# JuliaHealth/Thunderbolt.jl

Measured on AMD Instinct MI355X. Metric: element-integrations/sec + DoF-updates/sec, 10M-hex Q1 monodomain, higher is better.
Workload: dtype f64

## Files before the change

include/tbhip.h:

```cpp
#ifndef TBHIP_H
#define TBHIP_H
#include <stddef.h>
#include <stdint.h>

#ifdef __cplusplus
extern "C" {
#endif

typedef struct tb_device tb_device;
typedef struct tb_mesh tb_mesh;
typedef struct tb_pattern tb_pattern;
typedef struct tb_form tb_form;
typedef struct tb_locator tb_locator;
typedef struct tb_ecg tb_ecg;

enum {
    TB_OK = 0,
    TB_ERR_BAD_ARG = -1,
    TB_ERR_HIP = -2,
    TB_ERR_NEG_DETJ = -3,
    TB_ERR_PATTERN = -4,
    TB_ERR_UNSUPPORTED = -5,
    TB_ERR_NOMEM = -6
};
// ... 249 lines not shown
                     double *d_S);
int tb_gather_indexed(tb_device *dev, int64_t n, const double *d_vec, const int32_t *d_idx, double *d_out);
int tb_extract_diagonal(tb_pattern *pat, const double *d_nzval, double *d_diag);
int tb_scatter_add_indexed(tb_device *dev, int64_t n, const double *d_in, const int32_t *d_idx, double *d_vec);
int tb_scatter_indexed(tb_device *dev, int64_t n, const double *d_in, const int32_t *d_idx, double *d_vec);
typedef struct tb_comm tb_comm;
#define TB_COMM_ID_BYTES 128
enum { TB_REDUCE_SUM = 0, TB_REDUCE_MAX = 1 };
int tb_comm_unique_id(void *id128);
int tb_comm_create(tb_device *dev, const void *id128, int rank, int world_size, tb_comm **out);
int tb_comm_destroy(tb_comm *comm);
int tb_comm_rank_size(tb_comm *comm, int *rank, int *size);
int tb_comm_exchange(tb_comm *comm, int n_peers, const int32_t *peers, const int64_t *counts, const double *const *d_send, double *const *d_recv);
int tb_comm_allreduce(tb_comm *comm, double *d_buf, int64_t n, int op);
int tb_comm_exchange_begin(tb_comm *comm, int n_peers, const int32_t *peers, const int64_t *counts, const double *const *d_send, double *const *d_recv);
int tb_comm_exchange_end(tb_comm *comm);
typedef struct tb_graph tb_graph;
int tb_graph_begin(tb_device *dev);
int tb_graph_end(tb_device *dev, tb_graph **out);
int tb_graph_launch(tb_graph *graph, double t);
int tb_graph_node_count(tb_graph *graph, int *n);
int tb_graph_destroy(tb_graph *graph);
int tb_pattern_patch_stats(tb_pattern *pat, int64_t *out6);
int tb_pattern_spmv_plan(tb_pattern *pat, int64_t *out2);
int tb_spmv_mirror(tb_pattern *pat, const double *d_nzval);
int tb_spmv_csr_rows(tb_pattern *pat, const double *d_nzval, const double *d_x, int64_t n_rows, const int32_t *d_rows, double *d_out);
int tb_spmv_csr_dot(tb_pattern *pat, const double *d_nzval, const double *d_x, double *d_y, double *d_dot);
int tb_apply_zero_csr(tb_pattern *pat, double *d_nzval, double *d_f, const uint8_t *d_prescribed, double diag);
int tb_meandiag(tb_pattern *pat, const double *d_nzval, double *result);
int tb_max(tb_device *dev, int64_t n, const double *d_x, int64_t stride, double *result);

int tb_newmark_predict(tb_device *dev, int64_t n, double dt, double beta, double gamma, const double *d_u, const double *d_v, const double *d_a,
                       double *d_utilde, double *d_vtilde);
int tb_newmark_stage(tb_pattern *pat, const double *d_Mnz, double c, const double *d_u, const double *d_utilde, double *d_Jnz, double *d_r);
int tb_newmark_correct(tb_device *dev, int64_t n, double dt, double beta, double gamma, const double *d_u, const double *d_utilde, const double *d_vtilde,
                       double *d_a, double *d_v);
int tb_hermite_interpolate(tb_device *dev, int64_t n, double theta, double dt, int derivative, const double *d_u0, const double *d_v0, const double *d_u1,
                           const double *d_v1, double *d_out);

int tb_convert_f64_to_f32(tb_device *dev, int64_t n, const double *d_in, float *d_out);
int tb_convert_f32_to_f64(tb_device *dev, int64_t n, const float *d_in, double *d_out);
int tb_assemble_matrix_f32(tb_form *form, tb_pattern *pat, int strategy, double t, float *d_nzval);
int tb_assemble_matrix_pair_f32(tb_form *mass, tb_form *diffusion, tb_pattern *pat, int strategy, double t, float *d_nzval_mass, float *d_nzval_diffusion);
int tb_assemble_vector_f32(tb_form *form, int strategy, double t, float *d_b);
int tb_reaction_step_f32(tb_device *dev, int model, const double *params, int n_params, float *d_u, float *d_du, int64_t n_points, int n_states, int layout,
                         const float *d_x, int sdim, double t, double dt, int substeps, double threshold);
// ... 23 lines not shown
```

thunderbolt.jl_amd/_lib.py:

```python
import ctypes as C
import os
import subprocess

_HERE = os.path.dirname(os.path.abspath(__file__))
LIB_PATH = os.environ.get("TB_LIBTBHIP") or os.path.join(_HERE, "libtbhip.so")

TB_OK = 0
TB_ERR_BAD_ARG, TB_ERR_HIP, TB_ERR_NEG_DETJ, TB_ERR_PATTERN, TB_ERR_UNSUPPORTED, TB_ERR_NOMEM = -1, -2, -3, -4, -5, -6
TB_QUAD4, TB_HEX8, TB_TET4, TB_HEX27, TB_TET10 = 2, 3, 4, 5, 6
TB_STRATEGY_ATOMIC, TB_STRATEGY_PER_COLOR, TB_STRATEGY_ELEMENT, TB_STRATEGY_PATCH = 0, 1, 2, 3
TB_FORM_MASS, TB_FORM_DIFFUSION, TB_FORM_SOURCE, TB_FORM_HYPERELASTIC = 0, 1, 2, 3
TB_MATERIAL_HOLZAPFEL_OGDEN_2009 = 0
TB_BC_ROBIN, TB_BC_NORMAL_SPRING, TB_BC_PRESSURE, TB_BC_BENDING_SPRING, TB_BC_PRESSURE_FIELD = 0, 1, 2, 3, 4
TB_VOLUME_RSAFDQ2022, TB_VOLUME_HIRSCHVOGEL2017 = 0, 1
TB_COEF_CONST_SCALAR, TB_COEF_CONST_TENSOR, TB_COEF_FIELD_SCALAR = 0, 1, 2
TB_COEF_SPECTRAL_CONST, TB_COEF_SPECTRAL_FIELD, TB_COEF_TRANSVERSE_CONST = 3, 4, 5
TB_SRC_CONST, TB_SRC_NORM_PLUS_T, TB_SRC_COS_EXP, TB_SRC_TABULATED = 0, 1, 2, 3
TB_CELL_FHN, TB_CELL_ALIEV_PANFILOV, TB_CELL_PCG2019, TB_CELL_TT06, TB_CELL_FHN_HETEROGENEOUS, TB_CELL_ORD11 = 0, 1, 2, 3, 4, 5
TB_LAYOUT_SOA, TB_LAYOUT_AOS = 0, 1

c_dp = C.POINTER(C.c_double)
c_i32p = C.POINTER(C.c_int32)
c_i64p = C.POINTER(C.c_int64)
vp = C.c_void_p
# ... 147 lines not shown
    "tb_heat_matrix_f32": (C.c_int, [vp, C.c_int64, vp, vp, C.c_double, vp]),
    "tb_axpy_f32": (C.c_int, [vp, C.c_int64, C.c_double, vp, vp]),
    "tb_cg_solve_f32": (C.c_int, [vp, vp, vp, vp, C.c_double, C.c_double, C.c_int, C.c_int, vp, vp]),
    "tb_extract_diagonal": (C.c_int, [vp, vp, vp]),
    "tb_pattern_patch_stats": (C.c_int, [vp, vp]),
    "tb_comm_unique_id": (C.c_int, [vp]),
    "tb_comm_create": (C.c_int, [vp, vp, C.c_int, C.c_int, C.POINTER(vp)]),
    "tb_comm_destroy": (C.c_int, [vp]),
    "tb_comm_rank_size": (C.c_int, [vp, vp, vp]),
    "tb_comm_exchange": (C.c_int, [vp, C.c_int, vp, vp, vp, vp]),
    "tb_comm_allreduce": (C.c_int, [vp, vp, C.c_int64, C.c_int]),
    "tb_comm_exchange_begin": (C.c_int, [vp, C.c_int, vp, vp, vp, vp]),
    "tb_cgd_iteration": (C.c_int, [vp, vp, vp, vp, vp, vp, vp, vp]),
    "tb_cg1_update": (C.c_int, [vp, C.c_int64, vp, vp, vp, vp, vp, vp, vp, vp, vp]),
    "tb_cg1_fold": (C.c_int, [vp, vp]),
    "tb_cg1_iteration": (C.c_int, [vp, vp, vp, vp, vp, vp, vp, vp, vp, vp]),
    "tb_graph_begin": (C.c_int, [vp]),
    "tb_graph_end": (C.c_int, [vp, C.POINTER(vp)]),
    "tb_graph_launch": (C.c_int, [vp, C.c_double]),
    "tb_graph_node_count": (C.c_int, [vp, C.POINTER(C.c_int)]),
    "tb_graph_destroy": (C.c_int, [vp]),
    "tb_comm_exchange_end": (C.c_int, [vp]),
    "tb_pattern_spmv_plan": (C.c_int, [vp, vp]),
    "tb_scatter_add_indexed": (C.c_int, [vp, C.c_int64, vp, vp, vp]),
    "tb_scatter_indexed": (C.c_int, [vp, C.c_int64, vp, vp, vp]),
    "tb_spmv_csr_rows": (C.c_int, [vp, vp, vp, C.c_int64, vp, vp]),
    "tb_spmv_csr_dot": (C.c_int, [vp, vp, vp, vp, vp]),
    "tb_spmv_mirror": (C.c_int, [vp, vp]),
    "tb_apply_zero_csr": (C.c_int, [vp, vp, vp, vp, C.c_double]),
    "tb_meandiag": (C.c_int, [vp, vp, C.POINTER(C.c_double)]),
    "tb_max": (C.c_int, [vp, C.c_int64, vp, C.c_int64, C.POINTER(C.c_double)]),
    "tb_host_generate_grid_hex": (C.c_int, [C.c_int, C.c_int, C.c_int, c_dp, c_dp, c_dp, c_i32p]),
    "tb_host_generate_grid_tet": (C.c_int, [C.c_int, C.c_int, C.c_int, c_dp, c_dp, c_dp, c_i32p]),
    "tb_host_generate_grid_quad": (C.c_int, [C.c_int, C.c_int, c_dp, c_dp, c_dp, c_i32p]),
    "tb_host_perturb_nodes": (C.c_int, [C.c_int, C.c_int, C.c_int, C.c_double, c_dp]),
    "tb_host_close_dofs": (C.c_int64, [C.c_int, C.c_int, C.c_int64, C.c_int64, c_i32p, c_i32p]),
    "tb_host_build_pattern": (C.c_int64, [C.c_int64, C.c_int, c_i32p, C.c_int64, c_i64p, c_i32p]),
    "tb_host_locality_permutation": (C.c_int, [C.c_int, C.c_int64, c_dp, C.c_int64, c_i32p, C.c_int, c_i32p, C.c_int64, C.c_int, c_i32p, c_i32p, c_i32p]),
}


class TBError(RuntimeError):
    def __init__(self, code, msg):
        super().__init__("libtbhip error %d: %s" % (code, msg))
        self.code = code

# ... 42 lines not shown
```

thunderbolt.jl_amd/csrc/tb_api.cpp:

```cpp
#include <algorithm>
#include <mutex>
#include <cmath>
#include <cstdarg>
#include <cstring>

#include <omp.h>

#include "tb_internal.h"

namespace tb {

static thread_local std::string g_error;

void set_error(const char *fmt, ...)
{
    char buf[1024];
    va_list ap;
    va_start(ap, fmt);
    vsnprintf(buf, sizeof buf, fmt, ap);
    va_end(ap);
    g_error = buf;
}

static thread_local std::string g_last_kernel;
// ... 1268 lines not shown

int tb_pattern_spmv_plan(tb_pattern *pat, int64_t *out2)
{
    TB_REQUIRE(pat && out2, "tb_pattern_spmv_plan: NULL argument");
    TB_HIP(hipSetDevice(pat->mesh->dev->id));
    int rc = spmv_plans(pat);
    if (rc) return rc;
    out2[0] = pat->n_sig; out2[1] = pat->sig_entries;
    return TB_OK;
}

int tb_pattern_patch_stats(tb_pattern *pat, int64_t *out6)
{
    TB_REQUIRE(pat && out6, "tb_pattern_patch_stats: NULL argument");
    TB_HIP(hipSetDevice(pat->mesh->dev->id));
    int rc = ensure_patch_plans(pat->mesh, nullptr);
    if (rc) return rc;
    const PatchPlan *pp = pat->mesh->patches.get();
    out6[0] = pp->n_patches; out6[1] = pp->total_elems; out6[2] = pat->mesh->n_cells; out6[3] = pp->max_elems; out6[4] = pp->max_rows;
    out6[5] = pat->patch_fused ? (int64_t)pat->patch_fused->max_lds_entries * 8 : (pat->patch_mat ? (int64_t)pat->patch_mat->max_lds_entries * 8 : 0);
    return TB_OK;
}

int tb_gather_indexed(tb_device *dev, int64_t n, const double *d_vec, const int32_t *d_idx, double *d_out)
{
    TB_REQUIRE(dev && n >= 0 && ((d_vec && d_idx && d_out) || n == 0), "tb_gather_indexed: bad argument");
    TB_HIP(hipSetDevice(dev->id));
    return launch_gather_indexed(dev, n, d_vec, d_idx, d_out);
}

int tb_scatter_indexed(tb_device *dev, int64_t n, const double *d_in, const int32_t *d_idx, double *d_vec)
{
    TB_REQUIRE(dev && n >= 0 && ((d_vec && d_idx && d_in) || n == 0), "tb_scatter_indexed: bad argument");
    TB_HIP(hipSetDevice(dev->id));
    return launch_scatter_indexed(dev, n, d_in, d_idx, d_vec);
}

int tb_scatter_add_indexed(tb_device *dev, int64_t n, const double *d_in, const int32_t *d_idx, double *d_vec)
{
    TB_REQUIRE(dev && n >= 0 && ((d_vec && d_idx && d_in) || n == 0), "tb_scatter_add_indexed: bad argument");
    TB_HIP(hipSetDevice(dev->id));
    return launch_scatter_add_indexed(dev, n, d_in, d_idx, d_vec);
}

int tb_spmv_csr_rows(tb_pattern *pat, const double *d_nzval, const double *d_x, int64_t n_rows, const int32_t *d_rows, double *d_out)
{
// ... 50 lines not shown
```

thunderbolt.jl_amd/csrc/tb_assembly.hip:

```cpp
#include <hip/hip_runtime.h>

#include <cmath>
#include <cstring>
#include <type_traits>

#include "tb_elem.hpp"
#include "tb_forms.hpp"
#include "tb_hex8_sumfac.hpp"
#include "tb_internal.h"
#include "tb_math.hpp"

namespace tb {
using namespace tbk;

template <int NB> __host__ __device__ constexpr int sym_idx(int i, int j)
{
    return i <= j ? i * NB - (i * (i - 1)) / 2 + (j - i) : j * NB - (j * (j - 1)) / 2 + (i - j);
}

template <class E>
__device__ __forceinline__ void load_coords(const MeshView &m, int64_t cell, double (&x)[E::NV][3])
{
    int32_t nodes[E::NV];
    const int32_t *c = m.conn + cell * E::NV;
// ... 410 lines not shown
        double be[E::NB];
#pragma unroll
        for (int j = 0; j < E::NB; ++j) be[j] = 0.0;
        if (!element_source<E>(x, fa, cell, be)) flag_neg_detj(st, cell);
#pragma unroll
        for (int j = 0; j < E::NB; ++j)
            if (lr[j] != 0xFFFF) unsafeAtomicAdd(&acc[lr[j]], be[j]);
        if (!more) break;
        e = en; cell = celln;
#pragma unroll
        for (int a_ = 0; a_ < E::NV; ++a_) { x[a_][0] = xn[a_][0]; x[a_][1] = xn[a_][1]; x[a_][2] = xn[a_][2]; }
    }
    __syncthreads();
    for (int s = threadIdx.x; s < nrows; s += T) b[pv.row_dof[r0 + s]] = acc[s];
}

struct VecPatchView {
    const uint4 *hdr;
    const uint16_t *elem_ln;
    const int32_t *elem_cell;
    const double *pcoord;
    const int32_t *pdof;
    int max_nodes;
};

template <bool HALO, int KIND>
__global__ void __launch_bounds__(256, 4)
k_vector_hex8_patch(FormArgs fa, VecPatchView pv, double *__restrict__ b, Status *st)
{
    extern __shared__ double lds[];
    constexpr int T = 256, NX = 13;
    const int tid = threadIdx.x;
    const uint4 h = pv.hdr[blockIdx.x];
    const int64_t e0 = h.x, n0 = h.y;
    const int nrows = (int)(h.z & 0xffff), nnodes = (int)(h.z >> 16), ne = (int)h.w;
    double *acc = lds;
    double *xs = lds + pv.max_nodes;
    const uint4 *eln = (const uint4 *)pv.elem_ln + e0;
    const double *pc = pv.pcoord + 3 * n0;
    double xc[NX];
#pragma unroll
    for (int j = 0; j < NX; ++j) xc[j] = tid + j * T < 3 * nnodes ? pc[tid + j * T] : 0.0;
    const int32_t *pd = pv.pdof + n0;
    for (int k = tid; k < nnodes; k += T) acc[k] = 0.0;
#pragma unroll
    for (int j = 0; j < NX; ++j) if (tid + j * T < 3 * nnodes) xs[tid + j * T] = xc[j];
    for (int k = tid + NX * T; k < 3 * nnodes; k += T) xs[k] = pc[k];
    const double tv = source_time<KIND>(fa);
    __syncthreads();
#pragma unroll 1
    for (int ei = tid; HALO ? ei - tid < ne : ei < ne; ei += T) {
        const bool on = !HALO || ei < ne;
        double be[8];
        if (on) {
            const uint4 l4 = eln[ei];
            const uint32_t ln[8] = {l4.x & 0xffffu, l4.x >> 16, l4.y & 0xffffu, l4.y >> 16, l4.z & 0xffffu, l4.z >> 16, l4.w & 0xffffu, l4.w >> 16};
            double x[8][3];
#pragma unroll
            for (int a = 0; a < 8; ++a) {
                const double *px = xs + 3 * ln[a];
                x[a][0] = px[0]; x[a][1] = px[1]; x[a][2] = px[2];
            }
            int64_t cell = 0;
            if constexpr (KIND == TB_SRC_TABULATED) cell = pv.elem_cell[e0 + ei];
            if (!hex8_sf_source(x, [&](int q, const double(&xq)[3]) { return eval_source_k<KIND>(fa, tv, xq, cell, q, 8); }, be)) flag_neg_detj(st, pv.elem_cell[e0 + ei]);
        }
        auto scatter = [&]() {
            int es = ei;
            asm volatile("" : "+v"(es));
            const uint4 s4 = eln[es];
            const uint32_t sn[8] = {s4.x & 0xffffu, s4.x >> 16, s4.y & 0xffffu, s4.y >> 16, s4.z & 0xffffu, s4.z >> 16, s4.w & 0xffffu, s4.w >> 16};
#pragma unroll
            for (int a = 0; a < 8; ++a)
                if (!HALO || sn[a] < (uint32_t)nrows) unsafeAtomicAdd(acc + sn[a], be[a]);
        };
        if constexpr (HALO) {
#pragma unroll 1
            for (int w = 0; w < T / 64; ++w) {
                if (on && (tid >> 6) == w) scatter();
                __syncthreads();
            }
        } else {
            scatter();
        }
    }
    if constexpr (!HALO) __syncthreads();
    for (int k = tid; k < nrows; k += T) {
        if (HALO) b[pd[k]] = acc[k];
        else unsafeAtomicAdd(b + pd[k], acc[k]);
    }
}


static inline unsigned nblocks(int64_t n, int bs) { return (unsigned)((n + bs - 1) / bs); }

int ensure_emap(tb_pattern *p)
{
    if (p->d_emap) return TB_OK;
    tb_mesh *m = p->mesh;
    tb_device *dev = m->dev;
    const int64_t n = m->n_cells * m->ndpc;
    p->map64 = p->nnz >= (int64_t)0x7fffffff;
    const size_t bytes = (size_t)m->n_cells * m->ndpc * m->ndpc * (p->map64 ? 8 : 4);
    TB_HIP(hipMalloc(&p->d_emap, bytes));
    int rc = reset_status(dev);
    if (rc) return rc;
    if (p->map64)
        hipLaunchKernelGGL(k_build_emap<int64_t>, dim3(nblocks(n, 256)), dim3(256), 0, dev->stream, m->d_cell_dofs, m->n_cells,
                           m->ndpc, p->d_rowptr, p->d_colidx, (int64_t *)p->d_emap, dev->d_status);
    else
        hipLaunchKernelGGL(k_build_emap<int32_t>, dim3(nblocks(n, 256)), dim3(256), 0, dev->stream, m->d_cell_dofs, m->n_cells,
                           m->ndpc, p->d_rowptr, p->d_colidx, (int32_t *)p->d_emap, dev->d_status);
    TB_HIP(hipGetLastError());
// ... 916 lines not shown
        if (rc != TB_ERR_UNSUPPORTED) return rc;
        rc = reset_status(m->dev);
        if (rc) return rc;
    }
    if (m->field_kind == TB_HEX8 && f->qorder == 2) rc = run_matrix_form<Hex8<2>>(f, p, strategy, t, d_nz);
    else if (m->field_kind == TB_TET4 && f->qorder == 2) rc = run_matrix_form<Tet4<2>>(f, p, strategy, t, d_nz);
    else if (m->field_kind == TB_QUAD4 && f->qorder == 2) rc = run_matrix_form<Quad4<2>>(f, p, strategy, t, d_nz);
    else if (m->field_kind == TB_HEX27 && f->qorder == 3) rc = run_q2(f, p, strategy, t, d_nz, nullptr);
    else {
        set_error("matrix assembly: field kind %d with quadrature order %d not implemented", m->field_kind, f->qorder);
        return TB_ERR_UNSUPPORTED;
    }
    if (rc) return rc;
    return check_status(m->dev);
}

template <bool HALO, int KIND>
static int launch_vector_hex8_patch_inst(int64_t n_patches, size_t lds, tb_device *dev, const FormArgs &fa, const VecPatchView &pv, double *d_b)
{
    hipLaunchKernelGGL((k_vector_hex8_patch<HALO, KIND>), dim3((unsigned)n_patches), dim3(256), lds, dev->stream, fa, pv, d_b, dev->d_status);
    TB_HIP(hipGetLastError());
    return TB_OK;
}
template <int KIND>
static int launch_vector_hex8_patch(bool halo, int64_t n_patches, size_t lds, tb_device *dev, const FormArgs &fa, const VecPatchView &pv, double *d_b)
{
    return halo ? launch_vector_hex8_patch_inst<true, KIND>(n_patches, lds, dev, fa, pv, d_b) : launch_vector_hex8_patch_inst<false, KIND>(n_patches, lds, dev, fa, pv, d_b);
}

template <class E>
static int run_vector(tb_form *f, int strategy, double t, double *d_b)
{
    tb_mesh *m = f->mesh;
    tb_device *dev = m->dev;
    const MeshView mv = make_view(m);
    const FormArgs fa = make_args(f, t);
    static const bool legacy_vec = tune_env("TB_VECTOR_KERNEL") && !strcmp(tune_env("TB_VECTOR_KERNEL"), "legacy");
    if constexpr (std::is_same<E, Hex8<2>>::value) {
        if (!legacy_vec && !f->has_cellset && (strategy == TB_STRATEGY_PATCH || strategy == TB_STRATEGY_ATOMIC)) {
            const bool halo = strategy == TB_STRATEGY_PATCH;
            int rc = ensure_vec_patch_plan(m, halo);
            if (rc == TB_OK) {
                const VecPatchPlan *vp = m->vpatches[halo].get();
                const VecPatchView pv{(const uint4 *)vp->d_hdr, vp->d_elem_ln, vp->d_elem_cell, vp->d_pcoord, vp->d_pdof, vp->max_nodes};
                const size_t lds = (size_t)vp->max_nodes * 4 * sizeof(double);
                if (!halo) TB_HIP(hipMemsetAsync(d_b, 0, (size_t)m->ndofs * sizeof(double), dev->stream));
                rc = fa.src_kind == TB_SRC_CONST         ? launch_vector_hex8_patch<TB_SRC_CONST>(halo, vp->n_patches, lds, dev, fa, pv, d_b)
                     : fa.src_kind == TB_SRC_NORM_PLUS_T ? launch_vector_hex8_patch<TB_SRC_NORM_PLUS_T>(halo, vp->n_patches, lds, dev, fa, pv, d_b)
                     : fa.src_kind == TB_SRC_COS_EXP     ? launch_vector_hex8_patch<TB_SRC_COS_EXP>(halo, vp->n_patches, lds, dev, fa, pv, d_b)
                     : fa.src_kind == TB_SRC_TABULATED   ? launch_vector_hex8_patch<TB_SRC_TABULATED>(halo, vp->n_patches, lds, dev, fa, pv, d_b)
                                                         : TB_ERR_BAD_ARG;
                if (rc == TB_ERR_BAD_ARG) set_error("vector assembly: unknown source kind %d", fa.src_kind);
                return rc;
            }
            if (rc != TB_ERR_UNSUPPORTED) return rc;
        }
    }
    if (strategy == TB_STRATEGY_PATCH) {
        { int rc = ensure_patch_plans(m, nullptr); if (rc) return rc; }
        const PatchView pv = make_patch_view(m, nullptr);
        const int T = m->patches->threads;
        hipLaunchKernelGGL((k_vector_patch<E>), dim3((unsigned)m->patches->n_patches), dim3(T),
                           (size_t)m->patches->max_rows * sizeof(double), dev->stream, mv, fa, pv, d_b, dev->d_status);
        TB_HIP(hipGetLastError());
        return TB_OK;
    }
    if (strategy == TB_STRATEGY_ELEMENT) {
        if (!m->ea) { int rc = build_ea_plan(m); if (rc) return rc; }
        hipLaunchKernelGGL((k_vector_direct<E>), dim3(nblocks(m->n_cells, 256)), dim3(256), 0, dev->stream, mv, fa,
                           (const int32_t *)nullptr, m->n_cells, d_b, m->ea->d_ea, 2, dev->d_status);
        TB_HIP(hipGetLastError());
        hipLaunchKernelGGL(k_ea_gather, dim3(nblocks(m->ndofs, 256)), dim3(256), 0, dev->stream, m->ea->d_ptr, m->ea->d_src,
                           m->ea->d_ea, m->ndofs, d_b);
        TB_HIP(hipGetLastError());
        return TB_OK;
// ... 44 lines not shown
```

thunderbolt.jl_amd/csrc/tb_internal.h:

```cpp
#pragma once
#include <cstdio>
#include <cstdlib>
#include <ctime>
#include <hip/hip_runtime.h>

#include <cstdint>
#include <cstdio>
#include <cstdlib>
#include <memory>
#include <string>
#include <vector>

#include "tbhip.h"

namespace tb {

void set_error(const char *fmt, ...);
#ifdef TB_ABLATION
inline const char *tune_env(const char *name) { return getenv(name); }
#else
inline const char *tune_env(const char *) { return nullptr; }
#endif
void set_last_kernel(const char *fmt, ...);
const char *last_kernel();
// ... 109 lines not shown
    int max_lds_entries = 0, max_nodes = 0;
    int64_t nsig = 0;
    int64_t *d_node_ptr = nullptr;
    int32_t *d_pnode = nullptr;
    uint16_t *d_elem_ln = nullptr;
    uint32_t *d_elem_sig = nullptr;
    uint8_t *d_sigtab = nullptr;
    RowDesc *d_row_desc = nullptr;
    uint32_t *d_hdr = nullptr;
    double *d_pcoord = nullptr;
    uint8_t *d_rec = nullptr;
    int rec_stride = 0, rec_rm = 0, rec_nm = 0, rec_ne = 0;
};

struct VecPatchPlan {
    bool halo = false;
    int64_t n_patches = 0, total_elems = 0, total_nodes = 0;
    int max_nodes = 0, max_elems = 0;
    uint32_t *d_hdr = nullptr;
    uint16_t *d_elem_ln = nullptr;
    int32_t *d_elem_cell = nullptr;
    double *d_pcoord = nullptr;
    int32_t *d_pdof = nullptr;
};

constexpr int RED_SLOTS = 64, RED_STRIDE = 16, RED_GROUP = RED_SLOTS * RED_STRIDE;

}

struct tb_pattern;
struct tb_device {
    int id = 0;
    hipStream_t stream = nullptr;
    bool own_stream = true;
    int n_cu = 0;
    size_t hbm_bytes = 0;
    std::string name;
    tb::Status *d_status = nullptr;
    tb::Status *h_status = nullptr;
    bool defer_status = false;
    void *d_scratch = nullptr;
    size_t scratch_bytes = 0;
    double *d_slots = nullptr;
    double *d_readback = nullptr;
    double *d_tslot = nullptr;
    bool capturing = false, defer_before_capture = false, tslot_used = false;
    double *d_ecg_ws = nullptr;
// ... 254 lines not shown
```

thunderbolt.jl_amd/csrc/tb_plans.cpp:

```cpp
#include <algorithm>
#include <parallel/algorithm>
#include <cmath>
#include <cstdio>
#include <cstdlib>
#include <cstring>
#include <numeric>

#include "tb_internal.h"

namespace tb {

void dof_slots(const tb_mesh *m, std::vector<int64_t> &ptr, std::vector<int32_t> &src)
{
    const int64_t n = m->n_cells * m->ndpc;
    ptr.assign(m->ndofs + 1, 0);
    for (int64_t i = 0; i < n; ++i) ptr[m->h_cell_dofs[i] + 1]++;
    for (int64_t d = 0; d < m->ndofs; ++d) ptr[d + 1] += ptr[d];
    std::vector<int64_t> pos(ptr.begin(), ptr.end() - 1);
    src.resize(n);
    for (int64_t i = 0; i < n; ++i) src[pos[m->h_cell_dofs[i]]++] = (int32_t)i;
}

int build_ea_plan(tb_mesh *m)
{
// ... 849 lines not shown
        const bool too_big = rc == TB_ERR_UNSUPPORTED && p->patch_fused;
        free_patch_fused_plan(p);
        if (!too_big) return rc;
        if (fixed) { set_error("patch plan needs %lld B of LDS per patch (> 80 KiB): lower TB_PATCH_TILE / TB_PATCH_CELLS", (long long)bytes); return TB_ERR_UNSUPPORTED; }
        const int shrink = m->patches->shrink + 1, version = m->patches->version;
        free_patch_plan(m);
        rc = build_patch_plan(m, -shrink);
        if (rc) return rc;
        m->patches->shrink = shrink;
        m->patches->version = version + 1;
    }
    set_error("patch plan: could not fit the LDS budget");
    return TB_ERR_UNSUPPORTED;
}

}

namespace tb {

void free_vec_patch_plans(tb_mesh *m)
{
    for (auto &v : m->vpatches) {
        if (!v) continue;
        hipFree(v->d_hdr); hipFree(v->d_elem_ln); hipFree(v->d_elem_cell); hipFree(v->d_pcoord); hipFree(v->d_pdof);
        v.reset();
    }
}

int ensure_vec_patch_plan(tb_mesh *m, bool halo)
{
    if (m->vpatches[halo]) return TB_OK;
    if (m->ndpc != 8 || m->nverts != 8 || m->ncomp != 1) { set_error("vector patch plan: needs a scalar trilinear hexahedron field"); return TB_ERR_UNSUPPORTED; }
    PlanTimer timer("ensure_vec_patch_plan");
    int tile[3] = {8, 8, 8};
    if (const char *e = tune_env("TB_VPATCH_TILE")) {
        int a, b, c;
        if (sscanf(e, "%d,%d,%d", &a, &b, &c) == 3 && a > 0 && b > 0 && c > 0) { tile[0] = a; tile[1] = b; tile[2] = c; }
    }
    const int64_t nc = m->n_cells;
    std::vector<uint32_t> bucket((size_t)nc * 3);
    std::vector<std::pair<uint64_t, int32_t>> keyed(nc);
    int64_t Rv[3] = {1, 1, 1};
    {
        std::vector<double> cen((size_t)nc * 3), cext((size_t)nc * 3);
        double lo[3] = {1e300, 1e300, 1e300}, hi[3] = {-1e300, -1e300, -1e300}, hsum[3] = {0, 0, 0};
#pragma omp parallel for schedule(static) reduction(min : lo[:3]) reduction(max : hi[:3]) reduction(+ : hsum[:3])
        for (int64_t c = 0; c < nc; ++c) {
            double mn[3] = {1e300, 1e300, 1e300}, mx[3] = {-1e300, -1e300, -1e300}, sum[3] = {0, 0, 0};
            for (int a = 0; a < 8; ++a)
                for (int d = 0; d < 3; ++d) {
                    const double v = m->h_xyz[3 * (int64_t)m->h_conn[c * 8 + a] + d];
                    sum[d] += v; mn[d] = std::min(mn[d], v); mx[d] = std::max(mx[d], v);
                }
            double ext[3];
            hex_axis_extents(&m->h_xyz[0], &m->h_conn[c * 8], ext);
            for (int d = 0; d < 3; ++d) {
                cen[3 * c + d] = sum[d] / 8;
// ... 122 lines not shown
    }
    if (bad) { set_error("vector patch plan: dofs and vertices of the field are not in one-to-one correspondence"); return TB_ERR_UNSUPPORTED; }
    if ((int64_t)plan->max_nodes * 32 > 160 * 1024 / 3) {
        set_error("vector patch plan: a patch touches %d nodes (%d B of LDS, more than a third of a CU's 160 KiB)", plan->max_nodes, plan->max_nodes * 32);
        return TB_ERR_UNSUPPORTED;
    }
    if ((int64_t)ecell.size() >= (int64_t)0x7fffffff || (int64_t)pnode.size() >= (int64_t)0x7fffffff) { set_error("vector patch plan: too many instances for 32-bit offsets"); return TB_ERR_UNSUPPORTED; }
    plan->total_elems = (int64_t)ecell.size();
    plan->total_nodes = (int64_t)pnode.size();
    std::vector<double> pcoord(pnode.size() * 3);
#pragma omp parallel for schedule(static)
    for (int64_t k = 0; k < (int64_t)pnode.size(); ++k)
        for (int d = 0; d < 3; ++d) pcoord[3 * k + d] = m->h_xyz[3 * (int64_t)pnode[k] + d];
    if (getenv("TB_PLAN_VERBOSE"))
        fprintf(stderr, "[tbhip] vector patch plan (%s): %lld patches, %.3f instances per cell, %.3f patch nodes per dof, max %d instances / %d nodes per patch\n",
                halo ? "halo" : "own cells", (long long)np, (double)ecell.size() / (double)std::max<int64_t>(nc, 1), (double)pnode.size() / (double)std::max<int64_t>(m->ndofs, 1),
                plan->max_elems, plan->max_nodes);
    int rc = TB_OK;
    if (!rc) rc = upload(m->dev, hdr, &plan->d_hdr);
    if (!rc) rc = upload(m->dev, ln, &plan->d_elem_ln);
    if (!rc) rc = upload(m->dev, ecell, &plan->d_elem_cell);
    if (!rc) rc = upload(m->dev, pcoord, &plan->d_pcoord);
    if (!rc) rc = upload(m->dev, pdof, &plan->d_pdof);
    if (rc) { hipFree(plan->d_hdr); hipFree(plan->d_elem_ln); hipFree(plan->d_elem_cell); hipFree(plan->d_pcoord); hipFree(plan->d_pdof); return rc; }
    m->vpatches[halo] = std::move(plan);
    return TB_OK;
}

}
```

Before: 11.78 billion.

## Pack vector patch data into contiguous per-patch records staged into LDS

Builds a per-patch contiguous record (header, element local indices, node coordinates, dof ids) padded to a fixed stride, and adds a record kernel that loads the whole record in one pass of wide vector loads into registers, then stores it to LDS before the element loop. Element indices and dof ids are then read from LDS rather than global memory, which is meant to cut load latency and the number of scattered global reads per workgroup. The cost is extra device memory for padded records and larger LDS use per workgroup. The change also adds optional timestamp profiling under an ablation flag and some plan introspection APIs.

```diff
diff --git a/include/tbhip.h b/include/tbhip.h
--- a/include/tbhip.h
+++ b/include/tbhip.h
@@ -295,6 +295,10 @@
 int tb_graph_node_count(tb_graph *graph, int *n);
 int tb_graph_destroy(tb_graph *graph);
 int tb_pattern_patch_stats(tb_pattern *pat, int64_t *out6);
+int tb_mesh_vector_plan(tb_mesh *mesh, int halo, int64_t *out8);
+int tb_mesh_vector_plan_array(tb_mesh *mesh, int halo, int which, void *out, int64_t nbytes);
+int tb_vector_record_layout(int max_elems, int max_nodes, int64_t *out8);
+int tb_vector_records_fill(int max_elems, int max_nodes, int64_t n_patches, const uint32_t *hdr, const uint16_t *elem_ln, const double *pcoord, const int32_t *pdof, uint8_t *rec);
 int tb_pattern_spmv_plan(tb_pattern *pat, int64_t *out2);
 int tb_spmv_mirror(tb_pattern *pat, const double *d_nzval);
 int tb_spmv_csr_rows(tb_pattern *pat, const double *d_nzval, const double *d_x, int64_t n_rows, const int32_t *d_rows, double *d_out);
diff --git a/thunderbolt.jl_amd/_lib.py b/thunderbolt.jl_amd/_lib.py
--- a/thunderbolt.jl_amd/_lib.py
+++ b/thunderbolt.jl_amd/_lib.py
@@ -193,6 +193,10 @@
     "tb_graph_destroy": (C.c_int, [vp]),
     "tb_comm_exchange_end": (C.c_int, [vp]),
     "tb_pattern_spmv_plan": (C.c_int, [vp, vp]),
+    "tb_mesh_vector_plan": (C.c_int, [vp, C.c_int, vp]),
+    "tb_mesh_vector_plan_array": (C.c_int, [vp, C.c_int, C.c_int, vp, C.c_int64]),
+    "tb_vector_record_layout": (C.c_int, [C.c_int, C.c_int, vp]),
+    "tb_vector_records_fill": (C.c_int, [C.c_int, C.c_int, C.c_int64, vp, vp, vp, vp, vp]),
     "tb_scatter_add_indexed": (C.c_int, [vp, C.c_int64, vp, vp, vp]),
     "tb_scatter_indexed": (C.c_int, [vp, C.c_int64, vp, vp, vp]),
     "tb_spmv_csr_rows": (C.c_int, [vp, vp, vp, C.c_int64, vp, vp]),
diff --git a/thunderbolt.jl_amd/csrc/tb_api.cpp b/thunderbolt.jl_amd/csrc/tb_api.cpp
--- a/thunderbolt.jl_amd/csrc/tb_api.cpp
+++ b/thunderbolt.jl_amd/csrc/tb_api.cpp
@@ -1314,6 +1314,64 @@
     return TB_OK;
 }
 
+int tb_vector_record_layout(int max_elems, int max_nodes, int64_t *out8)
+{
+    TB_REQUIRE(max_elems >= 0 && max_nodes >= 0 && out8, "tb_vector_record_layout: bad argument");
+    const VecRecordLayout L = vec_record_layout(max_elems, max_nodes);
+    out8[0] = L.off_ln; out8[1] = L.off_coord; out8[2] = L.off_dof; out8[3] = L.stride; out8[4] = L.rec_ne; out8[5] = L.rec_nm;
+    out8[6] = vec_record_lds(L.rec_ne, L.rec_nm); out8[7] = vec_record_fits(max_elems, max_nodes) ? 1 : 0;
+    return TB_OK;
+}
+
+int tb_vector_records_fill(int max_elems, int max_nodes, int64_t n_patches, const uint32_t *hdr, const uint16_t *elem_ln, const double *pcoord, const int32_t *pdof, uint8_t *rec)
+{
+    TB_REQUIRE(max_elems >= 0 && max_nodes >= 0 && n_patches >= 0 && ((hdr && elem_ln && pcoord && pdof && rec) || n_patches == 0), "tb_vector_records_fill: bad argument");
+    for (int64_t q = 0; q < n_patches; ++q)
+        TB_REQUIRE((int64_t)hdr[4 * q + 3] <= max_elems && (int64_t)(hdr[4 * q + 2] >> 16) <= max_nodes, "tb_vector_records_fill: patch %lld exceeds the record's slots", (long long)q);
+    const VecRecordLayout L = vec_record_layout(max_elems, max_nodes);
+    memset(rec, 0, (size_t)n_patches * (size_t)L.stride);
+    fill_vec_records(L, n_patches, hdr, elem_ln, pcoord, pdof, rec);
+    return TB_OK;
+}
+
+int tb_mesh_vector_plan(tb_mesh *mesh, int halo, int64_t *out8)
+{
+    TB_REQUIRE(mesh && out8 && (halo == 0 || halo == 1), "tb_mesh_vector_plan: bad argument");
+    TB_HIP(hipSetDevice(mesh->dev->id));
+    int rc = ensure_vec_patch_plan(mesh, halo != 0);
+    if (rc) return rc;
+    const VecPatchPlan *vp = mesh->vpatches[halo].get();
+    out8[0] = vp->n_patches; out8[1] = vp->total_elems; out8[2] = vp->total_nodes; out8[3] = vp->max_elems; out8[4] = vp->max_nodes;
+    out8[5] = vp->d_rec ? vp->rec_stride : 0; out8[6] = vp->rec_ne; out8[7] = vp->rec_nm;
+    return TB_OK;
+}
+
+int tb_mesh_vector_plan_array(tb_mesh *mesh, int halo, int which, void *out, int64_t nbytes)
+{
+    TB_REQUIRE(mesh && out && (halo == 0 || halo == 1), "tb_mesh_vector_plan_array: bad argument");
+    TB_NO_CAPTURE(mesh->dev);
+    TB_HIP(hipSetDevice(mesh->dev->id));
+    int rc = ensure_vec_patch_plan(mesh, halo != 0);
+    if (rc) return rc;
+    const VecPatchPlan *vp = mesh->vpatches[halo].get();
+    const void *src = nullptr;
+    int64_t size = 0;
+    switch (which) {
+    case 0: src = vp->d_hdr; size = vp->n_patches * 16; break;
+    case 1: src = vp->d_elem_ln; size = vp->total_elems * 16; break;
+    case 2: src = vp->d_elem_cell; size = vp->total_elems * 4; break;
+    case 3: src = vp->d_pcoord; size = vp->total_nodes * 24; break;
+    case 4: src = vp->d_pdof; size = vp->total_nodes * 4; break;
+    case 5: src = vp->d_rec; size = vp->d_rec ? vp->n_patches * vp->rec_stride : 0; break;
+    default: TB_REQUIRE(false, "tb_mesh_vector_plan_array: which = %d (0 … 5)", which);
+    }
+    TB_REQUIRE(nbytes == size, "tb_mesh_vector_plan_array: array %d holds %lld B, not %lld", which, (long long)size, (long long)nbytes);
+    if (size == 0) return TB_OK;
+    TB_SYNC_STREAM(mesh->dev);
+    TB_HIP(hipMemcpy(out, src, (size_t)size, hipMemcpyDeviceToHost));
+    return TB_OK;
+}
+
 int tb_gather_indexed(tb_device *dev, int64_t n, const double *d_vec, const int32_t *d_idx, double *d_out)
 {
     TB_REQUIRE(dev && n >= 0 && ((d_vec && d_idx && d_out) || n == 0), "tb_gather_indexed: bad argument");
diff --git a/thunderbolt.jl_amd/csrc/tb_assembly.hip b/thunderbolt.jl_amd/csrc/tb_assembly.hip
--- a/thunderbolt.jl_amd/csrc/tb_assembly.hip
+++ b/thunderbolt.jl_amd/csrc/tb_assembly.hip
@@ -456,7 +456,18 @@
     const double *pcoord;
     const int32_t *pdof;
     int max_nodes;
+#ifdef TB_ABLATION
+    long long *prof;
+#endif
 };
+
+#ifdef TB_ABLATION
+#define TB_VST(k) do { if (pv.prof && tid == 0 && (blockIdx.x & 1023) == 7) pv.prof[(blockIdx.x >> 10) * 8 + (k)] = wall_clock64(); } while (0)
+#define TB_VST_LANDED(k, v) do { if (pv.prof) { asm volatile("" :: "v"(v)); TB_VST(k); } } while (0)
+#else
+#define TB_VST(k) do { } while (0)
+#define TB_VST_LANDED(k, v) do { } while (0)
+#endif
 
 template <bool HALO, int KIND>
 __global__ void __launch_bounds__(256, 4)
@@ -465,7 +476,9 @@
     extern __shared__ double lds[];
     constexpr int T = 256, NX = 13;
     const int tid = threadIdx.x;
+    TB_VST(0);
     const uint4 h = pv.hdr[blockIdx.x];
+    TB_VST_LANDED(1, h.x);
     const int64_t e0 = h.x, n0 = h.y;
     const int nrows = (int)(h.z & 0xffff), nnodes = (int)(h.z >> 16), ne = (int)h.w;
     double *acc = lds;
@@ -482,12 +495,16 @@
     for (int k = tid + NX * T; k < 3 * nnodes; k += T) xs[k] = pc[k];
     const double tv = source_time<KIND>(fa);
     __syncthreads();
+    TB_VST(2);
 #pragma unroll 1
     for (int ei = tid; HALO ? ei - tid < ne : ei < ne; ei += T) {
         const bool on = !HALO || ei < ne;
         double be[8];
         if (on) {
             const uint4 l4 = eln[ei];
+#ifdef TB_ABLATION
+            if (ei < 2 * T) TB_VST_LANDED(ei < T ? 3 : 4, l4.x);
+#endif
             const uint32_t ln[8] = {l4.x & 0xffffu, l4.x >> 16, l4.y & 0xffffu, l4.y >> 16, l4.z & 0xffffu, l4.z >> 16, l4.w & 0xffffu, l4.w >> 16};
             double x[8][3];
 #pragma unroll
@@ -519,10 +536,119 @@
         }
     }
     if constexpr (!HALO) __syncthreads();
+    TB_VST(5);
     for (int k = tid; k < nrows; k += T) {
+#ifdef TB_ABLATION
+        const int32_t d0 = pd[k];
+        if (k == tid) TB_VST_LANDED(6, d0);
+#endif
         if (HALO) b[pd[k]] = acc[k];
         else unsafeAtomicAdd(b + pd[k], acc[k]);
     }
+#ifdef TB_ABLATION
+    if (pv.prof) { __builtin_amdgcn_s_waitcnt(0); TB_VST(7); }
+#endif
+}
+
+struct VecRecordView {
+    const uint8_t *rec;
+    const int32_t *elem_cell;
+    int64_t stride;
+    int rec_ne, rec_nm;
+#ifdef TB_ABLATION
+    long long *prof;
+#endif
+};
+
+template <bool HALO, int KIND>
+__global__ void __launch_bounds__(256, 4)
+k_vector_hex8_record(FormArgs fa, VecRecordView pv, double *__restrict__ b, Status *st)
+{
+    extern __shared__ double lds[];
+    constexpr int T = 256, NI = 3, NC = 6;
+    static_assert(NI * T == VEC_REC_MAX_NE && NC * T * 2 == VEC_REC_MAX_NM * 3 && T * 4 == VEC_REC_MAX_NM, "a record is staged in one pass");
+    const int tid = threadIdx.x;
+    TB_VST(0);
+    const uint8_t *rec = pv.rec + (int64_t)blockIdx.x * pv.stride;
+    const int ne_s = pv.rec_ne, nc_s = pv.rec_nm * 3 / 2, nd_s = pv.rec_nm / 4;
+    const uint4 *gln = (const uint4 *)(rec + 16);
+    const double2 *gxc = (const double2 *)(gln + ne_s);
+    const int4 *gdf = (const int4 *)(gxc + nc_s);
+    double *acc = lds;
+    double *xs = lds + pv.rec_nm;
+    uint4 *sln = (uint4 *)(lds + 4 * (size_t)pv.rec_nm);
+    int32_t *sdf = (int32_t *)(sln + ne_s);
+    uint4 li[NI];
+    double2 xc[NC];
+#pragma unroll
+    for (int j = 0; j < NI; ++j) li[j] = tid + j * T < ne_s ? gln[tid + j * T] : make_uint4(0, 0, 0, 0);
+#pragma unroll
+    for (int j = 0; j < NC; ++j) xc[j] = tid + j * T < nc_s ? gxc[tid + j * T] : make_double2(0.0, 0.0);
+    const int4 df = tid < nd_s ? gdf[tid] : make_int4(0, 0, 0, 0);
+    const uint4 h = *(const uint4 *)rec;
+    for (int k = tid; k < pv.rec_nm; k += T) acc[k] = 0.0;
+#pragma unroll
+    for (int j = 0; j < NI; ++j) if (tid + j * T < ne_s) sln[tid + j * T] = li[j];
+#pragma unroll
+    for (int j = 0; j < NC; ++j) if (tid + j * T < nc_s) ((double2 *)xs)[tid + j * T] = xc[j];
+    if (tid < nd_s) ((int4 *)sdf)[tid] = df;
+    const int64_t e0 = h.x;
+    const int nrows = (int)(h.y & 0xffff), ne = (int)h.z;
+    const double tv = source_time<KIND>(fa);
+    TB_VST_LANDED(1, h.x);
+    __syncthreads();
+    TB_VST(2);
+#pragma unroll 1
+    for (int ei = tid; HALO ? ei - tid < ne : ei < ne; ei += T) {
+        const bool on = !HALO || ei < ne;
+        double be[8];
+        if (on) {
+            const uint4 l4 = sln[ei];
+#ifdef TB_ABLATION
+            if (ei < 2 * T) TB_VST_LANDED(ei < T ? 3 : 4, l4.x);
+#endif
+            const uint32_t ln[8] = {l4.x & 0xffffu, l4.x >> 16, l4.y & 0xffffu, l4.y >> 16, l4.z & 0xffffu, l4.z >> 16, l4.w & 0xffffu, l4.w >> 16};
+            double x[8][3];
+#pragma unroll
+            for (int a = 0; a < 8; ++a) {
+                const double *px = xs + 3 * ln[a];
+                x[a][0] = px[0]; x[a][1] = px[1]; x[a][2] = px[2];
+            }
+            int64_t cell = 0;
+            if constexpr (KIND == TB_SRC_TABULATED) cell = pv.elem_cell[e0 + ei];
+            if (!hex8_sf_source(x, [&](int q, const double(&xq)[3]) { return eval_source_k<KIND>(fa, tv, xq, cell, q, 8); }, be)) flag_neg_detj(st, pv.elem_cell[e0 + ei]);
+        }
+        auto scatter = [&]() {
+            int es = ei;
+            asm volatile("" : "+v"(es));
+            const uint4 s4 = sln[es];
+            const uint32_t sn[8] = {s4.x & 0xffffu, s4.x >> 16, s4.y & 0xffffu, s4.y >> 16, s4.z & 0xffffu, s4.z >> 16, s4.w & 0xffffu, s4.w >> 16};
+#pragma unroll
+            for (int a = 0; a < 8; ++a)
+                if (!HALO || sn[a] < (uint32_t)nrows) unsafeAtomicAdd(acc + sn[a], be[a]);
+        };
+        if constexpr (HALO) {
+#pragma unroll 1
+            for (int w = 0; w < T / 64; ++w) {
+                if (on && (tid >> 6) == w) scatter();
+                __syncthreads();
+            }
+        } else {
+            scatter();
+        }
+    }
+    if constexpr (!HALO) __syncthreads();
+    TB_VST(5);
+    for (int k = tid; k < nrows; k += T) {
+#ifdef TB_ABLATION
+        if (k == tid) TB_VST_LANDED(6, sdf[k]);
+#endif
+        if (HALO) b[sdf[k]] = acc[k];
+        else unsafeAtomicAdd(b + sdf[k], acc[k]);
+    }
+#ifdef TB_ABLATION
+    if (pv.prof) { __builtin_amdgcn_s_waitcnt(0); TB_VST(7); }
+#endif
 }
 
 
@@ -1485,11 +1611,52 @@
     TB_HIP(hipGetLastError());
     return TB_OK;
 }
-template <int KIND>
-static int launch_vector_hex8_patch(bool halo, int64_t n_patches, size_t lds, tb_device *dev, const FormArgs &fa, const VecPatchView &pv, double *d_b)
+template <bool HALO, int KIND>
+static int launch_vector_hex8_patch_inst(int64_t n_patches, size_t lds, tb_device *dev, const FormArgs &fa, const VecRecordView &pv, double *d_b)
+{
+    hipLaunchKernelGGL((k_vector_hex8_record<HALO, KIND>), dim3((unsigned)n_patches), dim3(256), lds, dev->stream, fa, pv, d_b, dev->d_status);
+    TB_HIP(hipGetLastError());
+    return TB_OK;
+}
+template <int KIND, class View>
+static int launch_vector_hex8_patch(bool halo, int64_t n_patches, size_t lds, tb_device *dev, const FormArgs &fa, const View &pv, double *d_b)
 {
     return halo ? launch_vector_hex8_patch_inst<true, KIND>(n_patches, lds, dev, fa, pv, d_b) : launch_vector_hex8_patch_inst<false, KIND>(n_patches, lds, dev, fa, pv, d_b);
 }
+template <class View>
+static int launch_vector_hex8_kind(bool halo, int64_t n_patches, size_t lds, tb_device *dev, const FormArgs &fa, const View &pv, double *d_b)
+{
+    int rc = fa.src_kind == TB_SRC_CONST         ? launch_vector_hex8_patch<TB_SRC_CONST>(halo, n_patches, lds, dev, fa, pv, d_b)
+             : fa.src_kind == TB_SRC_NORM_PLUS_T ? launch_vector_hex8_patch<TB_SRC_NORM_PLUS_T>(halo, n_patches, lds, dev, fa, pv, d_b)
+             : fa.src_kind == TB_SRC_COS_EXP     ? launch_vector_hex8_patch<TB_SRC_COS_EXP>(halo, n_patches, lds, dev, fa, pv, d_b)
+             : fa.src_kind == TB_SRC_TABULATED   ? launch_vector_hex8_patch<TB_SRC_TABULATED>(halo, n_patches, lds, dev, fa, pv, d_b)
+                                                 : TB_ERR_BAD_ARG;
+    if (rc == TB_ERR_BAD_ARG) set_error("vector assembly: unknown source kind %d", fa.src_kind);
+    return rc;
+}
+
+#ifdef TB_ABLATION
+static int report_vector_stamps(tb_device *dev, const long long *d_prof, int nprof, const char *kernel)
+{
+    std::vector<long long> h((size_t)nprof * 8);
+    TB_SYNC_STREAM(dev);
+    TB_HIP(hipMemcpy(h.data(), d_prof, h.size() * sizeof(long long), hipMemcpyDeviceToHost));
+    double ph[7] = {0, 0, 0, 0, 0, 0, 0};
+    int n = 0;
+    for (int w = 0; w < nprof; ++w) {
+        const long long *a = &h[(size_t)w * 8];
+        bool all = true;
+        for (int k = 0; k < 8; ++k) all = all && a[k];
+        if (!all) continue;
+        for (int k = 0; k < 7; ++k) ph[k] += (double)(a[k + 1] - a[k]) * 0.01;
+        ++n;
+    }
+    if (n) fprintf(stderr, "[tbhip] %s phases (us): header / staging loads back %.2f | first barrier %.2f | trip-1 indices back %.2f | trip 1, trip-2 indices back %.2f | "
+                           "trip 2, barrier %.2f | dof ids back %.2f | flush, drain %.2f | life %.2f  (n=%d)\n",
+                   kernel, ph[0] / n, ph[1] / n, ph[2] / n, ph[3] / n, ph[4] / n, ph[5] / n, ph[6] / n, (ph[0] + ph[1] + ph[2] + ph[3] + ph[4] + ph[5] + ph[6]) / n, n);
+    return TB_OK;
+}
+#endif
 
 template <class E>
 static int run_vector(tb_form *f, int strategy, double t, double *d_b)
@@ -1505,15 +1672,33 @@
             int rc = ensure_vec_patch_plan(m, halo);
             if (rc == TB_OK) {
                 const VecPatchPlan *vp = m->vpatches[halo].get();
-                const VecPatchView pv{(const uint4 *)vp->d_hdr, vp->d_elem_ln, vp->d_elem_cell, vp->d_pcoord, vp->d_pdof, vp->max_nodes};
-                const size_t lds = (size_t)vp->max_nodes * 4 * sizeof(double);
+                const char *sw = getenv("TB_VECTOR_KERNEL");
+                const bool record = vp->d_rec && !(sw && !strcmp(sw, "patch"));
+                VecPatchView pv{(const uint4 *)vp->d_hdr, vp->d_elem_ln, vp->d_elem_cell, vp->d_pcoord, vp->d_pdof, vp->max_nodes};
+                VecRecordView rv{vp->d_rec, vp->d_elem_cell, vp->rec_stride, vp->rec_ne, vp->rec_nm};
+#ifdef TB_ABLATION
+                static long long *d_prof = nullptr;
+                static int prof_cap = 0;
+                const int nprof = (int)(vp->n_patches >> 10) + 1;
+                if (getenv("TB_PROF_STAMPS") && !dev->capturing && nprof > prof_cap) {
+                    if (d_prof) TB_HIP(hipFree(d_prof));
+                    d_prof = nullptr; prof_cap = 0;
+                    TB_HIP(hipMalloc((void **)&d_prof, (size_t)nprof * 8 * sizeof(long long)));
+                    prof_cap = nprof;
+                }
+                const bool stamped = d_prof && !dev->capturing;
+                if (stamped) TB_HIP(hipMemsetAsync(d_prof, 0, (size_t)nprof * 8 * sizeof(long long), dev->stream));
+                pv.prof = rv.prof = stamped ? d_prof : nullptr;
+#endif
                 if (!halo) TB_HIP(hipMemsetAsync(d_b, 0, (size_t)m->ndofs * sizeof(double), dev->stream));
-                rc = fa.src_kind == TB_SRC_CONST         ? launch_vector_hex8_patch<TB_SRC_CONST>(halo, vp->n_patches, lds, dev, fa, pv, d_b)
-                     : fa.src_kind == TB_SRC_NORM_PLUS_T ? launch_vector_hex8_patch<TB_SRC_NORM_PLUS_T>(halo, vp->n_patches, lds, dev, fa, pv, d_b)
-                     : fa.src_kind == TB_SRC_COS_EXP     ? launch_vector_hex8_patch<TB_SRC_COS_EXP>(halo, vp->n_patches, lds, dev, fa, pv, d_b)
-                     : fa.src_kind == TB_SRC_TABULATED   ? launch_vector_hex8_patch<TB_SRC_TABULATED>(halo, vp->n_patches, lds, dev, fa, pv, d_b)
-                                                         : TB_ERR_BAD_ARG;
-                if (rc == TB_ERR_BAD_ARG) set_error("vector assembly: unknown source kind %d", fa.src_kind);
+                static const char *const kinds[] = {"const", "norm_plus_t", "cos_exp", "tabulated"};
+                const char *kname = fa.src_kind == TB_SRC_CONST ? kinds[0] : fa.src_kind == TB_SRC_NORM_PLUS_T ? kinds[1] : fa.src_kind == TB_SRC_COS_EXP ? kinds[2] : kinds[3];
+                set_last_kernel("%s<%s,%s>", record ? "k_vector_hex8_record" : "k_vector_hex8_patch", halo ? "halo" : "atomic", kname);
+                if (record) rc = launch_vector_hex8_kind(halo, vp->n_patches, (size_t)vec_record_lds(vp->rec_ne, vp->rec_nm), dev, fa, rv, d_b);
+                else rc = launch_vector_hex8_kind(halo, vp->n_patches, (size_t)vp->max_nodes * 4 * sizeof(double), dev, fa, pv, d_b);
+#ifdef TB_ABLATION
+                if (!rc && stamped) rc = report_vector_stamps(dev, d_prof, nprof, record ? "k_vector_hex8_record" : "k_vector_hex8_patch");
+#endif
                 return rc;
             }
             if (rc != TB_ERR_UNSUPPORTED) return rc;
diff --git a/thunderbolt.jl_amd/csrc/tb_internal.h b/thunderbolt.jl_amd/csrc/tb_internal.h
--- a/thunderbolt.jl_amd/csrc/tb_internal.h
+++ b/thunderbolt.jl_amd/csrc/tb_internal.h
@@ -155,7 +155,24 @@
     int32_t *d_elem_cell = nullptr;
     double *d_pcoord = nullptr;
     int32_t *d_pdof = nullptr;
-};
+    uint8_t *d_rec = nullptr;
+    int64_t rec_stride = 0;
+    int rec_ne = 0, rec_nm = 0;
+};
+
+struct VecRecordLayout {
+    int64_t off_ln = 16, off_coord = 0, off_dof = 0, stride = 0;
+    int rec_ne = 0, rec_nm = 0;
+};
+VecRecordLayout vec_record_layout(int max_elems, int max_nodes);
+inline int64_t vec_record_lds(int rec_ne, int rec_nm) { return (int64_t)rec_nm * 36 + (int64_t)rec_ne * 16; }
+constexpr int VEC_REC_MAX_NE = 768, VEC_REC_MAX_NM = 1024;
+inline bool vec_record_fits(int max_elems, int max_nodes)
+{
+    const int nm = (max_nodes + 3) & ~3;
+    return vec_record_lds(max_elems, nm) * 4 <= 160 * 1024 && max_elems <= VEC_REC_MAX_NE && nm <= VEC_REC_MAX_NM;
+}
+void fill_vec_records(const VecRecordLayout &L, int64_t n_patches, const uint32_t *hdr, const uint16_t *ln, const double *pcoord, const int32_t *pdof, uint8_t *rec);
 
 constexpr int RED_SLOTS = 64, RED_STRIDE = 16, RED_GROUP = RED_SLOTS * RED_STRIDE;
 
diff --git a/thunderbolt.jl_amd/csrc/tb_plans.cpp b/thunderbolt.jl_amd/csrc/tb_plans.cpp
--- a/thunderbolt.jl_amd/csrc/tb_plans.cpp
+++ b/thunderbolt.jl_amd/csrc/tb_plans.cpp
@@ -895,8 +895,35 @@
 {
     for (auto &v : m->vpatches) {
         if (!v) continue;
-        hipFree(v->d_hdr); hipFree(v->d_elem_ln); hipFree(v->d_elem_cell); hipFree(v->d_pcoord); hipFree(v->d_pdof);
+        hipFree(v->d_hdr); hipFree(v->d_elem_ln); hipFree(v->d_elem_cell); hipFree(v->d_pcoord); hipFree(v->d_pdof); hipFree(v->d_rec);
         v.reset();
+    }
+}
+
+VecRecordLayout vec_record_layout(int max_elems, int max_nodes)
+{
+    VecRecordLayout L;
+    L.rec_ne = max_elems;
+    L.rec_nm = (max_nodes + 3) & ~3;
+    L.off_ln = 16;
+    L.off_coord = L.off_ln + (int64_t)L.rec_ne * 16;
+    L.off_dof = L.off_coord + (int64_t)L.rec_nm * 24;
+    L.stride = (L.off_dof + (int64_t)L.rec_nm * 4 + 127) & ~(int64_t)127;
+    return L;
+}
+
+void fill_vec_records(const VecRecordLayout &L, int64_t n_patches, const uint32_t *hdr, const uint16_t *ln, const double *pcoord, const int32_t *pdof, uint8_t *rec)
+{
+#pragma omp parallel for schedule(static)
+    for (int64_t q = 0; q < n_patches; ++q) {
+        uint8_t *r = rec + q * L.stride;
+        const uint32_t e0 = hdr[4 * q], n0 = hdr[4 * q + 1], counts = hdr[4 * q + 2], ne = hdr[4 * q + 3];
+        const uint32_t nnodes = counts >> 16;
+        const uint32_t head[4] = {e0, counts, ne, 0};
+        memcpy(r, head, 16);
+        memcpy(r + L.off_ln, ln + (size_t)e0 * 8, (size_t)ne * 16);
+        memcpy(r + L.off_coord, pcoord + (size_t)n0 * 3, (size_t)nnodes * 24);
+        memcpy(r + L.off_dof, pdof + n0, (size_t)nnodes * 4);
     }
 }
 
@@ -906,6 +933,10 @@
     if (m->ndpc != 8 || m->nverts != 8 || m->ncomp != 1) { set_error("vector patch plan: needs a scalar trilinear hexahedron field"); return TB_ERR_UNSUPPORTED; }
     PlanTimer timer("ensure_vec_patch_plan");
     int tile[3] = {8, 8, 8};
+    if (const char *e = getenv("TB_PATCH_TILE")) {
+        int a, b, c;
+        if (sscanf(e, "%d,%d,%d", &a, &b, &c) == 3 && a > 0 && b > 0 && c > 0) { tile[0] = a; tile[1] = b; tile[2] = c; }
+    }
     if (const char *e = tune_env("TB_VPATCH_TILE")) {
         int a, b, c;
         if (sscanf(e, "%d,%d,%d", &a, &b, &c) == 3 && a > 0 && b > 0 && c > 0) { tile[0] = a; tile[1] = b; tile[2] = c; }
@@ -1074,7 +1105,21 @@
     if (!rc) rc = upload(m->dev, ecell, &plan->d_elem_cell);
     if (!rc) rc = upload(m->dev, pcoord, &plan->d_pcoord);
     if (!rc) rc = upload(m->dev, pdof, &plan->d_pdof);
-    if (rc) { hipFree(plan->d_hdr); hipFree(plan->d_elem_ln); hipFree(plan->d_elem_cell); hipFree(plan->d_pcoord); hipFree(plan->d_pdof); return rc; }
+    if (!rc && np > 0 && vec_record_fits(plan->max_elems, plan->max_nodes)) {
+        const VecRecordLayout L = vec_record_layout(plan->max_elems, plan->max_nodes);
+        std::vector<uint8_t> rec((size_t)np * (size_t)L.stride, 0);
+        fill_vec_records(L, np, hdr.data(), ln.data(), pcoord.data(), pdof.data(), rec.data());
+        rc = upload(m->dev, rec, &plan->d_rec);
+        plan->rec_stride = L.stride; plan->rec_ne = L.rec_ne; plan->rec_nm = L.rec_nm;
+        if (getenv("TB_PLAN_VERBOSE")) {
+            const double used = 16.0 * (double)np + 16.0 * (double)ecell.size() + 28.0 * (double)pnode.size();
+            fprintf(stderr, "[tbhip] vector patch records (%s): %lld B per patch (%d instance slots, %d node slots), %.1f MB in all, %.1f %% of it padding\n",
+                    halo ? "halo" : "own cells", (long long)L.stride, L.rec_ne, L.rec_nm, (double)np * (double)L.stride / 1e6, 100.0 * (1.0 - used / ((double)np * (double)L.stride)));
+        }
+    } else if (!rc && getenv("TB_PLAN_VERBOSE"))
+        fprintf(stderr, "[tbhip] vector patch records (%s): none, %lld B of LDS per workgroup leave fewer than four on a CU\n", halo ? "halo" : "own cells",
+                (long long)vec_record_lds(plan->max_elems, (plan->max_nodes + 3) & ~3));
+    if (rc) { hipFree(plan->d_hdr); hipFree(plan->d_elem_ln); hipFree(plan->d_elem_cell); hipFree(plan->d_pcoord); hipFree(plan->d_pdof); hipFree(plan->d_rec); return rc; }
     m->vpatches[halo] = std::move(plan);
     return TB_OK;
 }
```

Result: no change. 11.90 billion (median of 6 runs) (+1.0%).
